# J-Schoepplenberg/zero-packet

Measured on AMD Instinct MI355X. Metric: device-resident Mpkt/s + GB/s, PacketParser::parse, 64-1500B mix, higher is better.
Workload: dtype u8; 1 GPU; 16M IPv4 TCP/UDP/ICMPv4, U[64,1500]B (config 3); config=c3, frames_per_gpu=16777216, bytes_per_gpu=13113571179, job_frames=16777216, job_bytes=13113571179, parallelism=dp1 (independent shards, no collective)

## Files before the change

__graft_entry__.py:

```python
import importlib
import json
import os
import subprocess
import sys

ROOT = os.path.dirname(os.path.abspath(__file__))
PKG = os.path.join(ROOT, "zero-packet_amd")
CSRC = os.path.join(PKG, "csrc")
HIP_SOURCES = ["zp_parse.hip", "zp_parse_slots.hip", "zp_ctx.hip", "zp_gen.hip", "zp_fields.hip", "zp_ring.hip", "zp_build.hip",
               "zp_stats.hip"]
HOST_SOURCES = ["zp_readers.c"]
HIPCC = os.environ.get("HIPCC", "/opt/rocm/bin/hipcc")


def _run(cmd, cwd=ROOT):
    print("+", " ".join(cmd), flush=True)
    subprocess.run(cmd, cwd=cwd, check=True)


def _stale(target, sources):
    if not os.path.exists(target):
        return True
    t = os.path.getmtime(target)
    return any(os.path.getmtime(s) > t for s in sources)


def build(force=False):
    inc = os.path.join(ROOT, "include")
    deps = [os.path.join(CSRC, f) for f in os.listdir(CSRC)] + [
        os.path.join(inc, f) for f in os.listdir(inc)]
    hip_so = os.path.join(PKG, "libzp_hip.so")
    if force or _stale(hip_so, deps):
        objs = []
        for src in HIP_SOURCES:
            obj = os.path.join(CSRC, src.replace(".hip", ".o"))
            _run([HIPCC, "--offload-arch=gfx950", "-O3", "-std=c++17", "-fPIC",
                  "-Wall", "-c", os.path.join(CSRC, src), "-o", obj])
            objs.append(obj)
        for src in HOST_SOURCES:
            obj = os.path.join(CSRC, src.replace(".c", ".o"))
            _run(["gcc", "-O3", "-std=c11", "-Wall", "-Wextra", "-fPIC", "-c",
                  os.path.join(CSRC, src), "-o", obj])
# ... 83 lines not shown
```

include/zero_packet.h:

```cpp
#ifndef ZERO_PACKET_H
#define ZERO_PACKET_H

#include <stddef.h>
#include <stdint.h>

#ifdef __cplusplus
extern "C" {
#endif

#define ZP_ABI_VERSION 6

typedef enum zp_err {
    ZP_OK = 0,
    ZP_ERR_ETH_FRAME_TOO_SHORT = 1,
    ZP_ERR_ETH_SLICE_TOO_SHORT = 2,
    ZP_ERR_ETH_VLAN_TOO_SHORT = 3,
    ZP_ERR_ETH_QINQ_TOO_SHORT = 4,
    ZP_ERR_ETH_INVALID_QINQ = 5,
    ZP_ERR_ARP_TOO_SHORT = 6,
    ZP_ERR_ARP_INVALID_OPER = 7,
    ZP_ERR_IPV4_TOO_SHORT = 8,
    ZP_ERR_IPV4_VERSION = 9,
    ZP_ERR_IPV4_IHL_TOO_SHORT = 10,
    ZP_ERR_IPV4_HDR_TOO_LONG = 11,
// ... 90 lines not shown
        (((c >> 10) & 3u) + 1u) * 8u};
    uint32_t at = 0;
    for (int k = 0; k < ZP_EXT_SLOTS; ++k) x->off[k] = 0;
    for (int j = 0; j < 6; ++j) {
        const int k = order[j];
        if (r.flags & ZP_F_EXT_SLOT(k)) { x->off[k] = (uint16_t)at; at += len[k]; }
    }
    x->len = (uint16_t)at;
    x->final_nh = (uint8_t)((r.flags & ZP_F_TCP) ? 6 : (r.flags & ZP_F_UDP) ? 17
                          : (r.flags & ZP_F_ICMPV4) ? 1 : 58);
    x->reserved = 0;
}

typedef struct zp_rec_fields {
    uint32_t flags;
    uint8_t  err, eth_len, final_nh, inner_final_nh;
    uint32_t inner_off, l4_off;
} zp_rec_fields;

int zp_rec_decode(const zp_record* rec, const uint8_t* frame, uint64_t len,
                  const zp_ext_offsets* ext, zp_rec_fields* out);

int zp_abi_version(void);
const char* zp_err_str(int code);
const char* zp_last_error(void);

int zp_parse_batch_device(const uint8_t* arena, const uint64_t* offs,
                          const uint32_t* lens, uint64_t n,
                          zp_record* records, zp_ext_offsets* ext,
                          void* stream);

int zp_set_record_slots(int mode);
int zp_record_slots_state(void);

typedef struct zp_ctx zp_ctx;
zp_ctx* zp_ctx_create(int device, uint64_t chunk_bytes);
void    zp_ctx_destroy(zp_ctx* ctx);
int zp_parse_batch_host(zp_ctx* ctx, const uint8_t* arena, uint64_t arena_bytes,
                        const uint64_t* offs, const uint32_t* lens, uint64_t n,
                        zp_record* records, zp_ext_offsets* ext);
int zp_parse_batch_host_multi(zp_ctx* const* ctxs, int nctx, const uint8_t* arena,
                              uint64_t arena_bytes, const uint64_t* offs,
                              const uint32_t* lens, uint64_t n, zp_record* records,
                              zp_ext_offsets* ext);
int zp_parse_one(zp_ctx* ctx, const uint8_t* frame, uint64_t len,
                 zp_record* record, zp_ext_offsets ext[2]);
int zp_parse_one_config(zp_ctx* ctx, uint32_t idle_us);
int zp_device_current(void);

typedef enum zp_reader_kind {
    ZP_READER_ETHERNET = 0,
    ZP_READER_ARP = 1,
    ZP_READER_IPV4 = 2,
    ZP_READER_IPV6 = 3,
    ZP_READER_OPTIONS = 4,
    ZP_READER_ROUTING = 5,
    ZP_READER_FRAGMENT = 6,
    ZP_READER_AUTH = 7,
    ZP_READER_TCP = 8,
    ZP_READER_UDP = 9,
    ZP_READER_ICMPV4 = 10,
    ZP_READER_ICMPV6 = 11,
    ZP_READER_KIND_COUNT = 12
} zp_reader_kind;

typedef struct zp_reader_info {
// ... 204 lines not shown
```

zero-packet_amd/_lib.py:

```python
import ctypes
import os

HERE = os.path.dirname(os.path.abspath(__file__))
HIP_LIB = os.path.join(HERE, "libzp_hip.so")
HOST_LIB = os.path.join(HERE, "libzp_host.so")

_hip = None
_pyhip = None
_host = None

c_u8p = ctypes.c_void_p


def _sig(lib, name, res, args):
    f = getattr(lib, name)
    f.restype = res
    f.argtypes = args
    return f


def hip():
    global _hip
    if _hip is None:
        if not os.path.exists(HIP_LIB):
            raise RuntimeError(f"zero-packet_amd: HIP library missing ({HIP_LIB}); "
                               "run __graft_entry__.build() - there is no CPU fallback")
        lib = ctypes.CDLL(HIP_LIB)
        vp, u64, u32, i32 = ctypes.c_void_p, ctypes.c_uint64, ctypes.c_uint32, ctypes.c_int
        _sig(lib, "zp_abi_version", i32, [])
        _sig(lib, "zp_err_str", ctypes.c_char_p, [i32])
        _sig(lib, "zp_last_error", ctypes.c_char_p, [])
        _sig(lib, "zp_parse_batch_device", i32, [vp, vp, vp, u64, vp, vp, vp])
        _sig(lib, "zp_set_record_slots", i32, [i32])
        _sig(lib, "zp_record_slots_state", i32, [])
        _sig(lib, "zp_ctx_create", vp, [i32, u64])
        _sig(lib, "zp_ctx_destroy", None, [vp])
        _sig(lib, "zp_parse_batch_host", i32, [vp, vp, u64, vp, vp, u64, vp, vp])
        _sig(lib, "zp_parse_batch_host_multi", i32, [vp, i32, vp, u64, vp, vp, u64, vp, vp])
        _sig(lib, "zp_parse_one", i32, [vp, vp, u64, vp, vp])
        _sig(lib, "zp_parse_one_config", i32, [vp, u32])
        _sig(lib, "zp_device_current", i32, [])
        _sig(lib, "zp__one_test_hooks", i32, [vp, u32, u64, u32])
        _sig(lib, "zp__one_stats", i32, [vp, vp])
        _sig(lib, "zp_col_width", i32, [i32])
        _sig(lib, "zp_build_err_str", ctypes.c_char_p, [i32])
        _sig(lib, "zp_build_batch_device", i32, [vp, vp, vp, u64, vp, vp, vp, vp, vp])
        _sig(lib, "zp_extract_columns_device", i32, [vp, vp, vp, vp, u64, vp, vp])
        _sig(lib, "zp_parse_batch_columns_device", i32, [vp, vp, vp, u64, vp, vp, vp, vp])
        _sig(lib, "zp_stats_device", i32, [vp, u64, vp, vp])
        _sig(lib, "zp_probe_read_device", i32, [vp, u64, vp, vp])
        _sig(lib, "zp_probe_tiles_device", i32, [vp, u64, u64, vp, vp, vp, vp, vp])
        _sig(lib, "zp_probe_tiles_codes_device", i32, [vp, u64, u64, vp, vp, vp, vp, vp])
        _sig(lib, "zp_gen_lengths_device", i32, [i32, u64, u64, u64, vp, vp])
        _sig(lib, "zp_gen_frames_device", i32, [i32, u64, u64, u64, vp, vp, vp, vp])
        _sig(lib, "zp_reader_new", i32, [i32, vp, u64, vp])
        _sig(lib, "zp_internet_checksum", ctypes.c_uint16, [vp, u64, u32])
        _sig(lib, "zp_verify_internet_checksum", i32, [vp, u64, u32])
        _sig(lib, "zp_pseudo_header", u32, [vp, vp, u32, ctypes.c_uint8, u64])
        _sig(lib, "zp_rec_decode", i32, [vp, vp, u64, vp, vp])
        _hip = lib
    return _hip


def pyhip():
    global _pyhip
    if _pyhip is None:
        hip()
# ... 27 lines not shown
```

zero-packet_amd/csrc/zp_parse.hip:

```cpp

#include <hip/hip_runtime.h>
#include <stdint.h>
#include <string.h>
#include <stdio.h>
#include <stdlib.h>
#include <mutex>

#include "../../include/zero_packet.h"
#include "../../include/zero_packet_errstr.h"
#include "zp_cols.h"
#define ZP_WIN 112
#define ZP_WPE 5
#include "zp_stream.h"

#define ZP_WAVES 1
#define ZP_EXT_DENSE 32
#define ZP_K 1
#define ZP_SMALL_G 4
#define ZP_TAIL_G 4

#ifndef ZP_PARSE_SLOTS_TU
static __thread char g_last_error[256];

static void set_err(const char* what, hipError_t e) {
    snprintf(g_last_error, sizeof g_last_error, "%s: %s", what, hipGetErrorString(e));
}

extern "C" const char* zp_last_error(void) { return g_last_error; }
extern "C" __attribute__((visibility("hidden"))) char* zp__errbuf(void) { return g_last_error; }
extern "C" int zp_abi_version(void) { return ZP_ABI_VERSION; }
extern "C" const char* zp_err_str(int code) { return zp_err_string(code); }
#endif


__device__ __forceinline__ bool icmpv4_type_ok(uint32_t t) {
    const uint64_t m0 = (1ull << 0) | (1ull << 3) | (1ull << 4) | (1ull << 5) | (1ull << 8) |
                        (1ull << 9) | (1ull << 10) | (1ull << 11) | (1ull << 12) | (1ull << 13) |
                        (1ull << 14) | (1ull << 15) | (1ull << 16) | (1ull << 17) | (1ull << 18) |
                        (1ull << 30) | (1ull << 40) | (1ull << 42) | (1ull << 43);
    if (t < 64) return (m0 >> t) & 1;
    return t == 253 || t == 254;
}
__device__ __forceinline__ bool icmpv6_type_ok(uint32_t t) {
    if (t >= 1 && t <= 4) return true;
    if (t == 100 || t == 101 || t == 155 || t == 200 || t == 201) return true;
    return t >= 128 && t <= 153;
}

#define ZP_RSTRIDE (ZP_WIN / 4 + 1)
struct FrameView {
    const uint4* win;
    const uint32_t* reg;
    bool region;
    const uint8_t* g;
// ... 558 lines not shown

template <bool COLS, bool SYS = false, class L = WaveLds, bool SLOTS = false>
__device__ __forceinline__ void tile_finish(TileState& s, uint64_t n, int lane, L& lds,
                                            zp_record* __restrict__ records,
                                            zp_ext_offsets* __restrict__ ext,
                                            const ColPtrs& cols, uintptr_t sysbase = 0,
                                            zp_u32x2* sys_rec = nullptr) {
    constexpr bool TAILS = sizeof(lds.win) > sizeof(uint4) * ZP_WIN_CH * 64;
    static_assert(TAILS || !SYS, "the tail-free layout needs the region path");
    uint4* tail = TAILS ? &lds.win[0] + ZP_WIN_CH * 64 : nullptr;
    const uint8_t* g = (const uint8_t*)s.ga;
    const uint32_t fsum = lds.cend[s.rank & 63u] - ((s.rank & 63u) ? lds.cend[(s.rank & 63u) - 1u] : 0u);
    FrameView fv;
    fv.win = &lds.win[0];
    fv.g = g;
    fv.lane = s.rank & 63u;
    fv.shift = s.shift;
    fv.len = s.len;
    fv.wlen = s.wlen;
    fv.xc = make_uint4(0, 0, 0, 0);
    fv.xi = ~0u;
    fv.sysbase = SYS ? sysbase : 0;
    uint4 mytail;
    fv.region = !SYS;
    if (SYS) {
        mytail = tail[s.rank & 63u];
        fv.reg = nullptr;
    } else {
        static_assert(64 * ZP_RSTRIDE * 4 <= sizeof(L), "regions fit the wave's LDS");
        const uint32_t rk = s.rank & 63u;
        uint4 cell[ZP_WIN_CH];
#pragma unroll
        for (uint32_t c = 0; c < ZP_WIN_CH; ++c) cell[c] = lds.win[c * 64 + ((rk ^ c) & 63u)];
        mytail = tail[rk];
        wave_lds_fence();
        uint32_t* reg = (uint32_t*)&lds.win[0] + (uint32_t)lane * ZP_RSTRIDE;
#pragma unroll
        for (uint32_t c = 0; c < ZP_WIN_CH; ++c) {
            reg[4 * c] = cell[c].x; reg[4 * c + 1] = cell[c].y;
            reg[4 * c + 2] = cell[c].z; reg[4 * c + 3] = cell[c].w;
        }
        wave_lds_fence();
        fv.reg = reg;
    }
    Walk w;
    w.rec = zp_rec_full{};
    w.outer = make_uint4(0, 0, 0, 0);
    w.inner = make_uint4(0, 0, 0, 0);
    bool done = false;
    const Probe pr = probe_frame(fv);
    const bool probe = s.live && v4_probe(fv, pr);
    if (__builtin_popcountll(__ballot(probe)) >= (SYS ? 1 : 32)) {
        if (probe) done = fast_v4(fv, pr, w);
    }
    {
        const bool todo = s.live && !done;
        if (__ballot(todo) && !__ballot(todo && !fast_ip_probe(fv, pr))) {
            if (todo) done = fast_ip(fv, pr, w);
        }
    }
    if (__ballot(s.live && !done)) {
        if (s.live && !done) {
            w.rec = zp_rec_full{};
            walk_frame(fv, w);
        }
    }
    if (!s.live) return;
// ... 33 lines not shown
        const bool ho = (rec.flags & ZP_F_EXT) && !zp_chain_inline(rec),
                   hi = rec.flags & ZP_F_INNER_EXT;
        const uint64_t mo = __ballot(ho), mi = __ballot(hi);
        if (SYS) {
            if (ho) st_sys16(sysbase, (uintptr_t)(ext + p),
                             zp_u32x4{w.outer.x, w.outer.y, w.outer.z, w.outer.w});
            if (hi) st_sys16(sysbase, (uintptr_t)(ext + n + p),
                             zp_u32x4{w.inner.x, w.inner.y, w.inner.z, w.inner.w});
            if (ho || hi) asm volatile("s_waitcnt vmcnt(0)" ::: "memory");
        } else {
        if (mo && (ho || __builtin_popcountll(mo) >= ZP_EXT_DENSE))
            store_ext(ext, p, ho ? w.outer : make_uint4(0, 0, 0, 0));
        if (mi && (hi || __builtin_popcountll(mi) >= ZP_EXT_DENSE))
            store_ext(ext, n + p, hi ? w.inner : make_uint4(0, 0, 0, 0));
        }
    }
    if (COLS) {
        ViewReader rdr{fv};
        emit_columns(rdr, rec, rec.err == 0 && (rec.flags & ZP_F_ETHERNET), s.len, p, cols);
    }
}


#define ZP_KATTR __launch_bounds__(64 * ZP_WAVES) __attribute__((amdgpu_waves_per_eu(ZP_WPE)))
#define ZP_KATTR_COLS __launch_bounds__(64 * ZP_WAVES)
template <bool COLS, bool TINY = !COLS, class L = WaveLds, bool SLOTS = false>
__device__ __forceinline__ void parse_tile(uint64_t t, uint32_t len, uintptr_t ga, uint64_t n,
                                           int lane, L& lds,
                                           zp_record* __restrict__ records,
                                           zp_ext_offsets* __restrict__ ext,
                                           const ColPtrs& cols) {
    const uintptr_t fallback = (uintptr_t)&zp_safe_chunk;
    uint4* win = &lds.win[0];
    uint4* tail = &lds.win[0] + ZP_WIN_CH * 64;
    if (TINY && !__ballot(t * 64 + lane < n && len != 64u) &&
        tiny_tile(t, len, ga, n, lane, records, SLOTS))
        return;
    TileState s;
    tile_setup(s, t, len, ga, n, lane, lds);
    if (s.nitems <= ZP_SMALL_G) {
        uint4 vs[ZP_SMALL_G];
        uint32_t ks[ZP_SMALL_G];
        issue_group<ZP_SMALL_G>(0, s.nitems, s.cur, s.R, lane, fallback, vs, ks);
        consume_group<ZP_SMALL_G>(0, s.nitems, lane, vs, ks, win, tail, lds.cend, s.run);
    } else
    {
    uint4 va[ZP_G];
    uint32_t ka[ZP_G];
    issue_group<ZP_G>(0, s.nitems, s.cur, s.R, lane, fallback, va, ka);
    consume_group<ZP_G>(0, s.nitems, lane, va, ka, win, tail, lds.cend, s.run);
    for (uint32_t i0 = ZP_G; i0 < s.nitems; i0 += ZP_G) {
        if (s.nitems - i0 <= 2) {
            uint4 vt[2];
            uint32_t kt[2];
            issue_group<2>(i0, s.nitems, s.cur, s.R, lane, fallback, vt, kt);
            consume_group<2>(i0, s.nitems, lane, vt, kt, win, tail, lds.cend, s.run);
            break;
        }
        if (s.nitems - i0 <= ZP_TAIL_G) {
            uint4 vt[ZP_TAIL_G];
            uint32_t kt[ZP_TAIL_G];
            issue_group<ZP_TAIL_G>(i0, s.nitems, s.cur, s.R, lane, fallback, vt, kt);
            consume_group<ZP_TAIL_G>(i0, s.nitems, lane, vt, kt, win, tail, lds.cend, s.run);
            break;
        }
        issue_group<ZP_G>(i0, s.nitems, s.cur, s.R, lane, fallback, va, ka);
        consume_group<ZP_G>(i0, s.nitems, lane, va, ka, win, tail, lds.cend, s.run);
    }
    }
    wave_lds_fence();
    {
        const uint32_t r = s.rank & 63u;
        const uintptr_t org = ((uintptr_t)bperm(s.R.org_hi, r) << 32) | bperm(s.R.org_lo, r);
        s.ga = org + 16ull * bperm(s.R.pfx, r) + s.shift;
    }
    __builtin_amdgcn_s_setprio(0);
    tile_finish<COLS, false, L, SLOTS>(s, n, lane, lds, records, ext, cols);
}

template <bool COLS, bool SLOTS = false>
__device__ __forceinline__ void parse_tiles(const uint8_t* __restrict__ arena,
                                            const uint64_t* __restrict__ offs,
                                            const uint32_t* __restrict__ lens, uint64_t n,
                                            zp_record* __restrict__ records,
                                            zp_ext_offsets* __restrict__ ext,
                                            const ColPtrs& cols) {
    __shared__ WaveLds lds_all[ZP_WAVES];
    const int lane = threadIdx.x & 63;
    const int wid = threadIdx.x >> 6;
    WaveLds& lds = lds_all[wid];
    const uint64_t blk = blockIdx.x;
    for (uint32_t k = 0; k < ZP_K; ++k) {
        const uint64_t t = (blk * ZP_WAVES + wid) * ZP_K + k;
        if (t * 64 >= n) return;
        __builtin_amdgcn_s_setprio(1);
        if (k) wave_lds_fence();
        uint32_t len;
        uintptr_t ga;
        load_desc(arena, offs, lens, n, t, lane, len, ga);
        parse_tile<COLS, !COLS, WaveLds, SLOTS>(t, len, ga, n, lane, lds, records, ext, cols);
    }
}

#ifdef ZP_PARSE_SLOTS_TU
__global__ void ZP_KATTR
zp_parse_slots_kernel(const uint8_t* __restrict__ arena, const uint64_t* __restrict__ offs,
                      const uint32_t* __restrict__ lens, uint64_t n,
                      zp_record* __restrict__ records, zp_ext_offsets* __restrict__ ext) {
    const ColPtrs none{};
    parse_tiles<false, true>(arena, offs, lens, n, records, ext, none);
}
extern "C" __attribute__((visibility("hidden"))) hipError_t
zp__parse_slots_launch(uint64_t blocks, hipStream_t stream, const uint8_t* arena, const uint64_t* offs,
                       const uint32_t* lens, uint64_t n, zp_record* records, zp_ext_offsets* ext) {
    hipLaunchKernelGGL(zp_parse_slots_kernel, dim3((unsigned)blocks), dim3(64 * ZP_WAVES), 0, stream,
                       arena, offs, lens, n, records, ext);
    return hipGetLastError();
}
#else
extern "C" hipError_t zp__parse_slots_launch(uint64_t blocks, hipStream_t stream, const uint8_t* arena,
                                             const uint64_t* offs, const uint32_t* lens, uint64_t n,
                                             zp_record* records, zp_ext_offsets* ext);
__global__ void ZP_KATTR
zp_parse_kernel(const uint8_t* __restrict__ arena, const uint64_t* __restrict__ offs,
                const uint32_t* __restrict__ lens, uint64_t n,
                zp_record* __restrict__ records, zp_ext_offsets* __restrict__ ext) {
    const ColPtrs none{};
    parse_tiles<false>(arena, offs, lens, n, records, ext, none);
}

#define ZP_EXPAND_TILES 16
__global__ void __launch_bounds__(256) zp_rec_expand_kernel(zp_record* __restrict__ records, uint64_t n,
                                                             uint32_t* __restrict__ hint, uint32_t token) {
    const uint32_t lane = threadIdx.x & 63u;
    const uint64_t t0 = ((uint64_t)blockIdx.x * 4 + (threadIdx.x >> 6)) * ZP_EXPAND_TILES;
    const uint64_t full = n / 64;
    const uint32_t b3 = lane < ZP_EXPAND_TILES && t0 + lane < full
// ... 2 lines not shown
    if (!m) return;
    if (hint && lane == 0 && (threadIdx.x >> 6) == 0 && (blockIdx.x & 63u) == 0 &&
        __builtin_popcountll(m) * 4 >= 3 * ZP_EXPAND_TILES)
        __hip_atomic_store(hint, token, __ATOMIC_RELAXED, __HIP_MEMORY_SCOPE_SYSTEM);
    uint32_t c[ZP_EXPAND_TILES];
#pragma unroll
    for (int k = 0; k < ZP_EXPAND_TILES; ++k)
        c[k] = (m >> k) & 1u ? ((const uint8_t*)(records + (t0 + k) * 64))[lane] : 0u;
#pragma unroll
    for (int k = 0; k < ZP_EXPAND_TILES; ++k)
        if ((m >> k) & 1u)
            __builtin_nontemporal_store(code_rec(c[k]), (zp_u32x2*)(records + (t0 + k) * 64 + lane));
}

extern "C" __attribute__((visibility("hidden"))) int zp__rec_expand_launch(zp_record* records, uint64_t n,
                                                                         hipStream_t stream,
                                                                         uint32_t* hint, uint32_t token) {
    if (n < 64) return 0;
    const uint64_t per_block = 4 * ZP_EXPAND_TILES;
    hipLaunchKernelGGL(zp_rec_expand_kernel, dim3((unsigned)((n / 64 + per_block - 1) / per_block)),
                       dim3(256), 0, stream, records, n, hint, token);
    const hipError_t e = hipGetLastError();
    if (e != hipSuccess) { set_err("zp_rec_expand_kernel launch", e); return -2; }
    return 0;
}

#define ZP_SLOT_MIN_FRAMES (1ull << 21)
static int g_slot_mode = 0;
extern "C" int zp_set_record_slots(int mode) {
    if (mode < 0 || mode > 2) return -1;
    return __atomic_exchange_n(&g_slot_mode, mode, __ATOMIC_RELAXED);
}

#define ZP_SLOT_PROBE_EVERY 16
struct SlotState {
    std::mutex mu;
    uint32_t* word = nullptr;
    uint32_t* word_d = nullptr;
    hipEvent_t ev = nullptr;
    bool pending = false, decision = true, broken = false;
    uint64_t since = 0;
    uint64_t last_n = 0;
    uint32_t token = 0;
};
static SlotState g_slot_state[64];

extern "C" int zp_record_slots_state(void) {
    int dev = 0;
    if (hipGetDevice(&dev) != hipSuccess) { (void)hipGetLastError(); dev = 0; }
    SlotState& st = g_slot_state[dev & 63];
    std::lock_guard<std::mutex> guard(st.mu);
    return st.decision ? 1 : 0;
}

static bool slot_state_init(SlotState& st) {
    if (st.word || st.broken) return !st.broken;
    void* w = nullptr;
    if (hipHostMalloc(&w, 64, hipHostMallocMapped | hipHostMallocCoherent) != hipSuccess ||
        hipHostGetDevicePointer((void**)&st.word_d, w, 0) != hipSuccess ||
        hipEventCreateWithFlags(&st.ev, hipEventDisableTiming) != hipSuccess) {
        (void)hipGetLastError();
        st.broken = true;
        return false;
    }
    st.word = (uint32_t*)w;
    return true;
}

__global__ void ZP_KATTR_COLS
zp_parse_columns_kernel(const uint8_t* __restrict__ arena, const uint64_t* __restrict__ offs,
                        const uint32_t* __restrict__ lens, uint64_t n,
                        zp_record* __restrict__ records, zp_ext_offsets* __restrict__ ext,
                        ColPtrs cols) {
    parse_tiles<true>(arena, offs, lens, n, records, ext, cols);
}

extern "C" int zp_parse_batch_device(const uint8_t* arena, const uint64_t* offs,
                                     const uint32_t* lens, uint64_t n,
                                     zp_record* records, zp_ext_offsets* ext,
                                     void* stream) {
    if (n == 0) return 0;
    if (!arena || !offs || !lens || !records) {
        snprintf(g_last_error, sizeof g_last_error, "zp_parse_batch_device: null pointer");
        return -1;
    }
    const uint64_t per_block = 64ull * ZP_WAVES * ZP_K;
    const uint64_t blocks = (n + per_block - 1) / per_block;
    if (blocks > 0x7FFFFFFFull) {
        snprintf(g_last_error, sizeof g_last_error, "zp_parse_batch_device: batch too large");
        return -1;
    }
    const int mode = __atomic_load_n(&g_slot_mode, __ATOMIC_RELAXED);
    const hipStream_t st_h = (hipStream_t)stream;
    auto launch = [&](bool slots, uint32_t* hint, uint32_t token) -> int {
        hipError_t e;
        if (slots) {
            e = zp__parse_slots_launch(blocks, st_h, arena, offs, lens, n, records, ext);
        } else {
            hipLaunchKernelGGL(zp_parse_kernel, dim3((unsigned)blocks), dim3(64 * ZP_WAVES), 0,
                               st_h, arena, offs, lens, n, records, ext);
            e = hipGetLastError();
        }
        if (e != hipSuccess) { set_err("zp_parse_kernel launch", e); return -2; }
        return slots ? zp__rec_expand_launch(records, n, st_h, hint, token) : 0;
    };
    if (mode != 0 || n < ZP_SLOT_MIN_FRAMES) return launch(mode == 1, nullptr, 0);
    int dev = 0;
    if (hipGetDevice(&dev) != hipSuccess) { (void)hipGetLastError(); dev = 0; }
    SlotState& st = g_slot_state[dev & 63];
    std::lock_guard<std::mutex> guard(st.mu);
    hipStreamCaptureStatus cs = hipStreamCaptureStatusNone;
    if (hipStreamIsCapturing(st_h, &cs) != hipSuccess) { (void)hipGetLastError(); cs = hipStreamCaptureStatusActive; }
    if (cs != hipStreamCaptureStatusNone) return launch(st.decision, nullptr, 0);
    if (n != st.last_n) {
        st.last_n = n;
        st.since = 0;
        st.pending = false;
    }
    if (st.pending) {
        const hipError_t q = hipEventQuery(st.ev);
        if (q == hipSuccess) {
            st.decision = __atomic_load_n(st.word, __ATOMIC_ACQUIRE) == st.token;
            st.pending = false;
        } else {
            (void)hipGetLastError();
        }
    }
    if (st.pending || st.since++ % ZP_SLOT_PROBE_EVERY != 0 || !slot_state_init(st))
        return launch(st.decision, nullptr, 0);
    st.token = st.token + 1 ? st.token + 1 : 1;
    const int rc = launch(true, st.word_d, st.token);
    if (rc == 0 && hipEventRecord(st.ev, st_h) == hipSuccess) st.pending = true;
    else (void)hipGetLastError();
    return rc;
}

extern "C" int zp_parse_batch_columns_device(const uint8_t* arena, const uint64_t* offs,
                                             const uint32_t* lens, uint64_t n,
                                             zp_record* records, zp_ext_offsets* ext,
                                             void* const* cols, void* stream) {
    if (n == 0) return 0;
    if (!arena || !offs || !lens || !records || !cols) {
        snprintf(g_last_error, sizeof g_last_error, "zp_parse_batch_columns_device: null pointer");
        return -1;
    }
    ColPtrs c;
    for (int k = 0; k < ZP_COL_COUNT; ++k) c.p[k] = (uint8_t*)cols[k];
    const uint64_t per_block = 64ull * ZP_WAVES * ZP_K;
    const uint64_t blocks = (n + per_block - 1) / per_block;
    if (blocks > 0x7FFFFFFFull) {
        snprintf(g_last_error, sizeof g_last_error, "zp_parse_batch_columns_device: batch too large");
        return -1;
    }
    hipLaunchKernelGGL(zp_parse_columns_kernel, dim3((unsigned)blocks), dim3(64 * ZP_WAVES), 0,
                       (hipStream_t)stream, arena, offs, lens, n, records, ext, c);
    const hipError_t e = hipGetLastError();
    if (e != hipSuccess) { set_err("zp_parse_columns_kernel launch", e); return -2; }
    return 0;
}

#define ZP_ONE_BELL 0
#define ZP_ONE_REC 64
#define ZP_ONE_ACK 72
#define ZP_ONE_EXT 96
// ... 124 lines not shown
```

zero-packet_amd/csrc/zp_stream.h:

```cpp
#pragma once
#include <hip/hip_runtime.h>
#include <stdint.h>

#ifndef ZP_WIN
#define ZP_WIN 128
#endif
#define ZP_WIN_CH (ZP_WIN / 16)
static_assert(ZP_WIN % 16 == 0 && ZP_WIN <= 256, "ZP_WIN must be a multiple of 16, <= 256");
#define ZP_GIANT 65536u
#define ZP_G 8

#define ZP_GLOBAL __attribute__((address_space(1)))
typedef unsigned zp_u32x4 __attribute__((ext_vector_type(4)));
typedef unsigned zp_u32x2 __attribute__((ext_vector_type(2)));

__device__ __forceinline__ uint4 ldg16(uintptr_t a) {
    zp_u32x4 v = *(const ZP_GLOBAL zp_u32x4*)a;
    return make_uint4(v.x, v.y, v.z, v.w);
}
__device__ __forceinline__ uint32_t ldg4(uintptr_t a) { return *(const ZP_GLOBAL uint32_t*)a; }

__device__ __forceinline__ uint4 ld_stream(uintptr_t a) {
    zp_u32x4 v = __builtin_nontemporal_load((const ZP_GLOBAL zp_u32x4*)a);
    return make_uint4(v.x, v.y, v.z, v.w);
// ... 84 lines not shown
        s = sad16(d[i] & m, s);
    }
    return s;
}

struct Cursor {
    uint32_t rbase;
    uint32_t nz;
    uint64_t* starts;
};

struct Ranked {
    uint32_t org_lo, org_hi;
    uint32_t last;
    uint32_t pfx;
    uint32_t mid;
};

#define KEEP_IN (1u << 31)
#define KEEP_WIN (1u << 30)
#define KEEP_TAIL (1u << 29)
#define ZP_T4N 3
#define KEEP_T4 (1u << 28)
#define KEEP_T4D(k) (((k) >> 22) & 3u)
#define KEEP_MID (1u << 27)
#define KEEP_MIDB(k) (((k) >> 10) & 15u)
#define KEEP_CELL(k) ((k) & 0x3FFu)
#define KEEP_RANK(k) (((k) >> 16) & 63u)

__device__ __forceinline__ uint32_t bperm(uint32_t v, uint32_t r) {
    return (uint32_t)__builtin_amdgcn_ds_bpermute((int)(r << 2), (int)v);
}

#define ZP_STARTS 64
__device__ __forceinline__ void build_starts(uint32_t w0, const Cursor& c, const Ranked& R,
                                             int lane) {
    if ((uint32_t)lane < (uint32_t)ZP_STARTS) c.starts[lane] = 0;
    __builtin_amdgcn_fence(__ATOMIC_RELEASE, "wavefront");
    __builtin_amdgcn_wave_barrier();
    __builtin_amdgcn_fence(__ATOMIC_ACQUIRE, "wavefront");
    const uint32_t it = R.pfx >> 6;
    if ((uint32_t)lane < c.nz && it >= w0 && it < w0 + (uint32_t)ZP_STARTS)
        __hip_atomic_fetch_or(&c.starts[it - w0], 1ull << (R.pfx & 63u), __ATOMIC_RELAXED,
                              __HIP_MEMORY_SCOPE_WAVEFRONT);
    __builtin_amdgcn_fence(__ATOMIC_RELEASE, "wavefront");
    __builtin_amdgcn_wave_barrier();
    __builtin_amdgcn_fence(__ATOMIC_ACQUIRE, "wavefront");
}

template <int G, bool T4 = false>
__device__ __forceinline__ void issue_group(uint32_t i0, uint32_t nitems, Cursor& c,
                                            const Ranked& R, int lane, uintptr_t fallback,
                                            uint4 (&v)[G], uint32_t (&keep)[G]) {
    uintptr_t a[G];
    static_assert(ZP_STARTS % G == 0 && G % 2 == 0 && ZP_STARTS <= 64,
                  "group size must be even and divide ZP_STARTS");
    if ((i0 & (ZP_STARTS - 1u)) == 0 && i0 < nitems) build_starts(i0, c, R, lane);
    uint64_t Fq[G];
    zp_u32x4 m[G / 2];
    const zp_u32x4* sp = (const zp_u32x4*)&c.starts[i0 & (ZP_STARTS - 1u)];
#pragma unroll
    for (int q = 0; q < G / 2; ++q) m[q] = sp[q];
#pragma unroll
    for (int q = 0; q < G; ++q) {
        const uint32_t lo = (q & 1) ? m[q / 2].z : m[q / 2].x;
        const uint32_t hi = (q & 1) ? m[q / 2].w : m[q / 2].y;
        const uint64_t fu = ((uint64_t)(uint32_t)__builtin_amdgcn_readfirstlane(hi) << 32) |
// ... 35 lines not shown
__device__ __forceinline__ void retire_group(const uint4 (&v)[G]) {
#pragma unroll
    for (int q = 0; q < G; ++q) asm volatile("" ::"v"(v[q].x), "v"(v[q].y), "v"(v[q].z), "v"(v[q].w));
}

template <int G, bool T4 = false>
__device__ __forceinline__ void consume_group(uint32_t i0, uint32_t nitems, int lane,
                                              const uint4 (&v)[G], const uint32_t (&keep)[G],
                                              uint4* win, uint4* tail, uint32_t* cend,
                                              uint32_t& run, uint4* t4 = nullptr,
                                              uint32_t* cmid = nullptr) {
#pragma unroll
    for (int q = 0; q < G; ++q) {
        const uint32_t i = i0 + q;
        if (i >= nitems) continue;
        const uint32_t k = keep[q];
        if (k & KEEP_WIN) win[KEEP_CELL(k)] = v[q];
        if (T4 && (k & KEEP_T4)) t4[KEEP_RANK(k) * ZP_T4N + KEEP_T4D(k)] = v[q];
        uint32_t part = sad16(v[q].x, 0u);
        part = sad16(v[q].y, part);
        part = sad16(v[q].z, part);
        part = sad16(v[q].w, part);
        const uint32_t P = wave_scan(k & KEEP_IN ? part : 0u);
        if (k & KEEP_TAIL) {
            if (tail != nullptr) tail[KEEP_RANK(k)] = v[q];
            cend[KEEP_RANK(k)] = run + P;
        }
        if (T4 && (k & KEEP_MID)) cmid[KEEP_RANK(k)] = run + P - part + range_sum(v[q], 0u, KEEP_MIDB(k));
        run += rdl(P, 63);
    }
    retire_group(v);
}

struct WaveLds {
    uint4 win[(ZP_WIN_CH + 1) * 64];
    uint32_t cend[64];
    uint64_t starts[ZP_STARTS];
};

struct TileState {
    uint64_t tile;
    uintptr_t ga;
    uint32_t len, shift, wlen, rank;
    bool live, giant;
    uint32_t nitems;
    uint64_t ranked;
    Ranked R;
    Cursor cur;
    uint32_t run;
};

template <class L>
__device__ __forceinline__ void tile_setup(TileState& s, uint64_t tile, uint32_t len,
                                           uintptr_t ga, uint64_t n, int lane, L& lds,
                                           bool win_only = false, uint32_t mark = ~0u) {
    s.tile = tile;
    s.ga = ga;
    s.len = len;
    s.live = tile * 64 + lane < n;
    s.shift = (uint32_t)(ga & 15);
    s.wlen = len < ZP_WIN - s.shift ? len : ZP_WIN - s.shift;
    s.giant = len > ZP_GIANT;
    const uint32_t span = s.giant || (win_only && len + s.shift > ZP_WIN) ? (uint32_t)ZP_WIN
                                                                          : len + s.shift;
    const uint32_t nch = len >= 64 ? (span + 15) >> 4 : 0u;
    const uint64_t M = __ballot(nch > 0);
    s.ranked = M;
    s.rank = __builtin_amdgcn_mbcnt_hi((uint32_t)(M >> 32),
                                       __builtin_amdgcn_mbcnt_lo((uint32_t)M, 0u));
    const uint32_t incl = wave_scan(nch);
    const uint32_t pfx = incl - nch;
    const uint32_t T = rdl(incl, 63);
    s.nitems = (T + 63) >> 6;
    const uint32_t nz = (uint32_t)__builtin_popcountll(M);
    const uint32_t dst = nch ? s.rank : nz + ((uint32_t)lane - s.rank);
    const uintptr_t org = (ga & ~(uintptr_t)15) - 16ull * pfx;
    const int a = (int)(dst << 2);
    s.R.org_lo = (uint32_t)__builtin_amdgcn_ds_permute(a, (int)(uint32_t)org);
    s.R.org_hi = (uint32_t)__builtin_amdgcn_ds_permute(a, (int)(uint32_t)(org >> 32));
    s.R.last = (uint32_t)__builtin_amdgcn_ds_permute(a, (int)(incl - 1));
    s.R.pfx = (uint32_t)__builtin_amdgcn_ds_permute(a, (int)pfx);
    const uint32_t mc = mark != ~0u && nch ? (s.shift + mark) >> 4 : ~0u;
    const uint32_t mid = mc < nch ? ((pfx + mc) << 4) | ((s.shift + mark) & 15u) : ~0u;
    s.R.mid = (uint32_t)__builtin_amdgcn_ds_permute(a, (int)mid);
    s.cur.rbase = ~0u;
    s.cur.nz = nz;
    s.cur.starts = &lds.starts[0];
    s.run = 0;
}

__device__ __forceinline__ void wave_lds_fence() {
    __builtin_amdgcn_fence(__ATOMIC_RELEASE, "wavefront");
    __builtin_amdgcn_wave_barrier();
    __builtin_amdgcn_fence(__ATOMIC_ACQUIRE, "wavefront");
}

__device__ __forceinline__ void load_desc(const uint8_t* arena, const uint64_t* offs,
                                          const uint32_t* lens, uint64_t n, uint64_t tile,
                                          int lane, uint32_t& len, uintptr_t& ga) {
    const uint64_t p = tile * 64 + lane;
    const uint64_t pc = p < n ? p : n - 1;
    const uint32_t l = lens[pc];
    const uint64_t o = offs[pc];
    len = p < n ? l : 0u;
    ga = (uintptr_t)arena + (p < n ? o : 0);
}
```

Before: 8470 Mpkt/s.

## Add tail-free LDS parse variants selected by a sampled batch profile

Adds two kernel variants that drop the per-wave LDS tail buffer, with window sizes 112 or 128 and a smaller starts array. Each frame's last 16-byte chunk is then taken from the neighbouring window cell or reloaded from global memory. A sampling profile kernel checks whether frames are packed contiguously and how often IPv6 extension headers appear, and the host uses that to pick a layout on later calls. The smaller LDS footprint is meant to raise occupancy, at the cost of extra global loads for tails, an extra profiling launch, and more dispatch complexity.

```diff
diff --git a/__graft_entry__.py b/__graft_entry__.py
--- a/__graft_entry__.py
+++ b/__graft_entry__.py
@@ -7,7 +7,7 @@
 ROOT = os.path.dirname(os.path.abspath(__file__))
 PKG = os.path.join(ROOT, "zero-packet_amd")
 CSRC = os.path.join(PKG, "csrc")
-HIP_SOURCES = ["zp_parse.hip", "zp_parse_slots.hip", "zp_ctx.hip", "zp_gen.hip", "zp_fields.hip", "zp_ring.hip", "zp_build.hip",
+HIP_SOURCES = ["zp_parse.hip", "zp_parse_slots.hip", "zp_parse_tf.hip", "zp_parse_tf128.hip", "zp_ctx.hip", "zp_gen.hip", "zp_fields.hip", "zp_ring.hip", "zp_build.hip",
                "zp_stats.hip"]
 HOST_SOURCES = ["zp_readers.c"]
 HIPCC = os.environ.get("HIPCC", "/opt/rocm/bin/hipcc")
diff --git a/include/zero_packet.h b/include/zero_packet.h
--- a/include/zero_packet.h
+++ b/include/zero_packet.h
@@ -146,6 +146,8 @@
 
 int zp_set_record_slots(int mode);
 int zp_record_slots_state(void);
+int zp_set_parse_layout(int mode);
+int zp_parse_layout_state(void);
 
 typedef struct zp_ctx zp_ctx;
 zp_ctx* zp_ctx_create(int device, uint64_t chunk_bytes);
diff --git a/zero-packet_amd/_lib.py b/zero-packet_amd/_lib.py
--- a/zero-packet_amd/_lib.py
+++ b/zero-packet_amd/_lib.py
@@ -33,6 +33,8 @@
         _sig(lib, "zp_parse_batch_device", i32, [vp, vp, vp, u64, vp, vp, vp])
         _sig(lib, "zp_set_record_slots", i32, [i32])
         _sig(lib, "zp_record_slots_state", i32, [])
+        _sig(lib, "zp_set_parse_layout", i32, [i32])
+        _sig(lib, "zp_parse_layout_state", i32, [])
         _sig(lib, "zp_ctx_create", vp, [i32, u64])
         _sig(lib, "zp_ctx_destroy", None, [vp])
         _sig(lib, "zp_parse_batch_host", i32, [vp, vp, u64, vp, vp, u64, vp, vp])
diff --git a/zero-packet_amd/csrc/zp_parse.hip b/zero-packet_amd/csrc/zp_parse.hip
--- a/zero-packet_amd/csrc/zp_parse.hip
+++ b/zero-packet_amd/csrc/zp_parse.hip
@@ -9,9 +9,17 @@
 #include "../../include/zero_packet.h"
 #include "../../include/zero_packet_errstr.h"
 #include "zp_cols.h"
+#ifndef ZP_WIN
 #define ZP_WIN 112
+#endif
 #define ZP_WPE 5
+#ifndef ZP_DESC_NT
+#define ZP_DESC_NT 0
+#endif
 #include "zp_stream.h"
+#if defined(ZP_PARSE_SLOTS_TU) || defined(ZP_PARSE_TF_TU)
+#define ZP_PARSE_KERNEL_TU 1
+#endif
 
 #define ZP_WAVES 1
 #define ZP_EXT_DENSE 32
@@ -19,7 +27,7 @@
 #define ZP_SMALL_G 4
 #define ZP_TAIL_G 4
 
-#ifndef ZP_PARSE_SLOTS_TU
+#ifndef ZP_PARSE_KERNEL_TU
 static __thread char g_last_error[256];
 
 static void set_err(const char* what, hipError_t e) {
@@ -644,7 +652,18 @@
         uint4 cell[ZP_WIN_CH];
 #pragma unroll
         for (uint32_t c = 0; c < ZP_WIN_CH; ++c) cell[c] = lds.win[c * 64 + ((rk ^ c) & 63u)];
-        mytail = tail[rk];
+        if (TAILS) {
+            mytail = tail[rk];
+        } else {
+            const uint32_t nr = (rk + 1u) & 63u;
+            const uint4 ncell = lds.win[nr];
+            const uintptr_t nA = ((((uintptr_t)bperm(s.R.org_hi, nr)) << 32) | bperm(s.R.org_lo, nr)) +
+                                 16ull * bperm(s.R.pfx, nr);
+            const uintptr_t lastc = (s.ga + s.len - 1u) & ~(uintptr_t)15;
+            const bool nxt = rk + 1u < s.cur.nz && nA == lastc;
+            const bool need = s.live && s.len >= 64 && !s.giant && ((s.len + s.shift) & 15u) != 0u;
+            mytail = nxt ? ncell : (need ? ldg16(lastc) : make_uint4(0, 0, 0, 0));
+        }
         wave_lds_fence();
         uint32_t* reg = (uint32_t*)&lds.win[0] + (uint32_t)lane * ZP_RSTRIDE;
 #pragma unroll
@@ -744,7 +763,8 @@
                                            const ColPtrs& cols) {
     const uintptr_t fallback = (uintptr_t)&zp_safe_chunk;
     uint4* win = &lds.win[0];
-    uint4* tail = &lds.win[0] + ZP_WIN_CH * 64;
+    uint4* tail = sizeof(lds.win) > sizeof(uint4) * ZP_WIN_CH * 64 ? &lds.win[0] + ZP_WIN_CH * 64
+                                                                  : nullptr;
     if (TINY && !__ballot(t * 64 + lane < n && len != 64u) &&
         tiny_tile(t, len, ga, n, lane, records, SLOTS))
         return;
@@ -790,17 +810,17 @@
     tile_finish<COLS, false, L, SLOTS>(s, n, lane, lds, records, ext, cols);
 }
 
-template <bool COLS, bool SLOTS = false>
+template <bool COLS, bool SLOTS = false, class L = WaveLds>
 __device__ __forceinline__ void parse_tiles(const uint8_t* __restrict__ arena,
                                             const uint64_t* __restrict__ offs,
                                             const uint32_t* __restrict__ lens, uint64_t n,
                                             zp_record* __restrict__ records,
                                             zp_ext_offsets* __restrict__ ext,
                                             const ColPtrs& cols) {
-    __shared__ WaveLds lds_all[ZP_WAVES];
+    __shared__ L lds_all[ZP_WAVES];
     const int lane = threadIdx.x & 63;
     const int wid = threadIdx.x >> 6;
-    WaveLds& lds = lds_all[wid];
+    L& lds = lds_all[wid];
     const uint64_t blk = blockIdx.x;
     for (uint32_t k = 0; k < ZP_K; ++k) {
         const uint64_t t = (blk * ZP_WAVES + wid) * ZP_K + k;
@@ -809,12 +829,27 @@
         if (k) wave_lds_fence();
         uint32_t len;
         uintptr_t ga;
-        load_desc(arena, offs, lens, n, t, lane, len, ga);
-        parse_tile<COLS, !COLS, WaveLds, SLOTS>(t, len, ga, n, lane, lds, records, ext, cols);
-    }
-}
-
-#ifdef ZP_PARSE_SLOTS_TU
+        load_desc<ZP_DESC_NT != 0>(arena, offs, lens, n, t, lane, len, ga);
+        parse_tile<COLS, !COLS, L, SLOTS>(t, len, ga, n, lane, lds, records, ext, cols);
+    }
+}
+
+#if defined(ZP_PARSE_TF_TU)
+__global__ void ZP_KATTR
+ZP_TF_KERNEL(const uint8_t* __restrict__ arena, const uint64_t* __restrict__ offs,
+             const uint32_t* __restrict__ lens, uint64_t n,
+             zp_record* __restrict__ records, zp_ext_offsets* __restrict__ ext) {
+    const ColPtrs none{};
+    parse_tiles<false, false, WaveLdsTailFree>(arena, offs, lens, n, records, ext, none);
+}
+extern "C" __attribute__((visibility("hidden"))) hipError_t
+ZP_TF_LAUNCH(uint64_t blocks, hipStream_t stream, const uint8_t* arena, const uint64_t* offs,
+             const uint32_t* lens, uint64_t n, zp_record* records, zp_ext_offsets* ext) {
+    hipLaunchKernelGGL(ZP_TF_KERNEL, dim3((unsigned)blocks), dim3(64 * ZP_WAVES), 0, stream,
+                       arena, offs, lens, n, records, ext);
+    return hipGetLastError();
+}
+#elif defined(ZP_PARSE_SLOTS_TU)
 __global__ void ZP_KATTR
 zp_parse_slots_kernel(const uint8_t* __restrict__ arena, const uint64_t* __restrict__ offs,
                       const uint32_t* __restrict__ lens, uint64_t n,
@@ -883,37 +918,143 @@
     return __atomic_exchange_n(&g_slot_mode, mode, __ATOMIC_RELAXED);
 }
 
+static int g_layout_mode = 0;
+extern "C" int zp_set_parse_layout(int mode) {
+    if (mode == -1) return __atomic_load_n(&g_layout_mode, __ATOMIC_RELAXED);
+    if (mode < 0 || mode > 3) return -1;
+    return __atomic_exchange_n(&g_layout_mode, mode, __ATOMIC_RELAXED);
+}
+extern "C" hipError_t zp__parse_tf_launch(uint64_t blocks, hipStream_t stream, const uint8_t* arena,
+                                          const uint64_t* offs, const uint32_t* lens, uint64_t n,
+                                          zp_record* records, zp_ext_offsets* ext);
+extern "C" hipError_t zp__parse_tf128_launch(uint64_t blocks, hipStream_t stream, const uint8_t* arena,
+                                             const uint64_t* offs, const uint32_t* lens, uint64_t n,
+                                             zp_record* records, zp_ext_offsets* ext);
+
+#define ZP_PROFILE_STRIDE 64
+#define ZP_PROFILE_PER_WAVE 4
+#define ZP_PROFILE_WAVES 16
+#define ZP_PROFILE_ACC_WORDS 8
+#define ZP_PROFILE_OUT 4
+__global__ void __launch_bounds__(64 * ZP_PROFILE_WAVES)
+zp_batch_profile_kernel(const uint8_t* __restrict__ arena, const uint64_t* __restrict__ offs,
+                        const uint32_t* __restrict__ lens, uint64_t n, uint32_t* __restrict__ acc,
+                        uint32_t* __restrict__ out, uint32_t token) {
+    __shared__ unsigned long long sums[ZP_PROFILE_WAVES][2];
+    const uint32_t lane = threadIdx.x & 63u, wave = threadIdx.x >> 6;
+    unsigned long long A = 0, B = 0;
+#pragma unroll
+    for (int j = 0; j < ZP_PROFILE_PER_WAVE; ++j) {
+        const uint64_t smp = ((uint64_t)blockIdx.x * ZP_PROFILE_WAVES + wave) * ZP_PROFILE_PER_WAVE + j;
+        const uint64_t p0 = smp * ZP_PROFILE_STRIDE * 64;
+        if (p0 >= n) break;
+        const uint64_t p = p0 + lane;
+        const bool live = p < n;
+        const uint64_t pc = live ? p : n - 1;
+        const uint64_t o = offs[pc];
+        const uint32_t len = lens[pc];
+        const bool pair = lane < 63 && p + 1 < n;
+        const uint64_t o1 = offs[pair ? p + 1 : pc];
+        const bool packed = !__ballot(pair && o + len != o1);
+        const uint8_t* f = arena + o;
+        auto at = [&](uint32_t i) -> uint32_t { return live && i < len && i < 32u ? f[i] : 0x100u; };
+        const uint32_t t0 = at(12) << 8 | at(13);
+        const uint32_t hl = t0 == 0x8100 ? 18u : t0 == 0x88A8 ? 22u : 14u;
+        const uint32_t et = hl == 14u ? t0 : at(hl - 2) << 8 | at(hl - 1);
+        const uint32_t nh = at(hl + 6);
+        const bool v6ext = et == 0x86DD && (nh == 0 || nh == 43 || nh == 44 || nh == 51 || nh == 60);
+        A += (1ull << 32) | (packed ? 1ull : 0ull);
+        B += ((unsigned long long)__builtin_popcountll(__ballot(live)) << 32) |
+             (unsigned long long)__builtin_popcountll(__ballot(v6ext));
+    }
+    if (lane == 0) { sums[wave][0] = A; sums[wave][1] = B; }
+    __syncthreads();
+    if (threadIdx.x != 0) return;
+    A = B = 0;
+    for (int w = 0; w < ZP_PROFILE_WAVES; ++w) { A += sums[w][0]; B += sums[w][1]; }
+    unsigned long long* a64 = (unsigned long long*)(acc + (token & 3u) * ZP_PROFILE_ACC_WORDS);
+    uint32_t* done = (uint32_t*)(a64 + 2);
+    atomicAdd(a64, A);
+    atomicAdd(a64 + 1, B);
+    __threadfence();
+    if (atomicAdd(done, 1u) + 1u != gridDim.x) return;
+    __threadfence();
+    A = atomicExch(a64, 0ull);
+    B = atomicExch(a64 + 1, 0ull);
+    atomicExch(done, 0u);
+    uint64_t* o64 = (uint64_t*)(out + ZP_PROFILE_OUT);
+    __hip_atomic_store(o64, (uint64_t)A, __ATOMIC_RELAXED, __HIP_MEMORY_SCOPE_SYSTEM);
+    __hip_atomic_store(o64 + 1, (uint64_t)B, __ATOMIC_RELAXED, __HIP_MEMORY_SCOPE_SYSTEM);
+    __hip_atomic_store(out + ZP_PROFILE_OUT + 4, token, __ATOMIC_RELEASE, __HIP_MEMORY_SCOPE_SYSTEM);
+}
+
 #define ZP_SLOT_PROBE_EVERY 16
-struct SlotState {
+#define ZP_PROFILE_V6EXT_DEN 2
+struct BatchProfile {
     std::mutex mu;
     uint32_t* word = nullptr;
     uint32_t* word_d = nullptr;
+    uint32_t* acc_d = nullptr;
     hipEvent_t ev = nullptr;
     bool pending = false, decision = true, broken = false;
+    bool probed_codes = false, probed_layout = false;
+    int layout = 1;
     uint64_t since = 0;
     uint64_t last_n = 0;
     uint32_t token = 0;
 };
-static SlotState g_slot_state[64];
-
-extern "C" int zp_record_slots_state(void) {
+static BatchProfile g_profile[64];
+
+static void profile_poll(BatchProfile& st) {
+    if (!st.pending) return;
+    if (hipEventQuery(st.ev) != hipSuccess) {
+        (void)hipGetLastError();
+        return;
+    }
+    st.pending = false;
+    if (st.probed_codes) st.decision = __atomic_load_n(st.word, __ATOMIC_ACQUIRE) == st.token;
+    if (st.probed_layout &&
+        __atomic_load_n(st.word + ZP_PROFILE_OUT + 4, __ATOMIC_ACQUIRE) == st.token) {
+        uint64_t s[2];
+        memcpy(s, st.word + ZP_PROFILE_OUT, sizeof s);
+        const uint64_t tiles = s[0] >> 32, packed = s[0] & 0xFFFFFFFFull;
+        const uint64_t frames = s[1] >> 32, exts = s[1] & 0xFFFFFFFFull;
+        st.layout = packed != tiles ? 1 : exts * ZP_PROFILE_V6EXT_DEN >= frames ? 3 : 2;
+    }
+}
+
+static BatchProfile& profile_here(void) {
     int dev = 0;
     if (hipGetDevice(&dev) != hipSuccess) { (void)hipGetLastError(); dev = 0; }
-    SlotState& st = g_slot_state[dev & 63];
+    return g_profile[dev & 63];
+}
+
+extern "C" int zp_record_slots_state(void) {
+    BatchProfile& st = profile_here();
     std::lock_guard<std::mutex> guard(st.mu);
+    profile_poll(st);
     return st.decision ? 1 : 0;
 }
-
-static bool slot_state_init(SlotState& st) {
+extern "C" int zp_parse_layout_state(void) {
+    BatchProfile& st = profile_here();
+    std::lock_guard<std::mutex> guard(st.mu);
+    profile_poll(st);
+    return st.layout;
+}
+
+static bool profile_init(BatchProfile& st) {
     if (st.word || st.broken) return !st.broken;
     void* w = nullptr;
     if (hipHostMalloc(&w, 64, hipHostMallocMapped | hipHostMallocCoherent) != hipSuccess ||
         hipHostGetDevicePointer((void**)&st.word_d, w, 0) != hipSuccess ||
+        hipMalloc((void**)&st.acc_d, 4 * ZP_PROFILE_ACC_WORDS * sizeof(uint32_t)) != hipSuccess ||
+        hipMemset(st.acc_d, 0, 4 * ZP_PROFILE_ACC_WORDS * sizeof(uint32_t)) != hipSuccess ||
         hipEventCreateWithFlags(&st.ev, hipEventDisableTiming) != hipSuccess) {
         (void)hipGetLastError();
         st.broken = true;
         return false;
     }
+    memset(w, 0, 64);
     st.word = (uint32_t*)w;
     return true;
 }
@@ -942,11 +1083,16 @@
         return -1;
     }
     const int mode = __atomic_load_n(&g_slot_mode, __ATOMIC_RELAXED);
+    const int lmode = __atomic_load_n(&g_layout_mode, __ATOMIC_RELAXED);
     const hipStream_t st_h = (hipStream_t)stream;
-    auto launch = [&](bool slots, uint32_t* hint, uint32_t token) -> int {
+    auto launch = [&](bool slots, int layout, uint32_t* hint, uint32_t token) -> int {
         hipError_t e;
         if (slots) {
             e = zp__parse_slots_launch(blocks, st_h, arena, offs, lens, n, records, ext);
+        } else if (layout == 2) {
+            e = zp__parse_tf_launch(blocks, st_h, arena, offs, lens, n, records, ext);
+        } else if (layout == 3) {
+            e = zp__parse_tf128_launch(blocks, st_h, arena, offs, lens, n, records, ext);
         } else {
             hipLaunchKernelGGL(zp_parse_kernel, dim3((unsigned)blocks), dim3(64 * ZP_WAVES), 0,
                                st_h, arena, offs, lens, n, records, ext);
@@ -955,32 +1101,37 @@
         if (e != hipSuccess) { set_err("zp_parse_kernel launch", e); return -2; }
         return slots ? zp__rec_expand_launch(records, n, st_h, hint, token) : 0;
     };
-    if (mode != 0 || n < ZP_SLOT_MIN_FRAMES) return launch(mode == 1, nullptr, 0);
-    int dev = 0;
-    if (hipGetDevice(&dev) != hipSuccess) { (void)hipGetLastError(); dev = 0; }
-    SlotState& st = g_slot_state[dev & 63];
+    if ((mode != 0 && lmode != 0) || n < ZP_SLOT_MIN_FRAMES)
+        return launch(mode == 1, lmode ? lmode : 1, nullptr, 0);
+    BatchProfile& st = profile_here();
     std::lock_guard<std::mutex> guard(st.mu);
+    auto decided = [&](void) -> int {
+        return launch(mode ? mode == 1 : st.decision, lmode ? lmode : st.layout, nullptr, 0);
+    };
     hipStreamCaptureStatus cs = hipStreamCaptureStatusNone;
     if (hipStreamIsCapturing(st_h, &cs) != hipSuccess) { (void)hipGetLastError(); cs = hipStreamCaptureStatusActive; }
-    if (cs != hipStreamCaptureStatusNone) return launch(st.decision, nullptr, 0);
+    if (cs != hipStreamCaptureStatusNone) return decided();
     if (n != st.last_n) {
         st.last_n = n;
         st.since = 0;
         st.pending = false;
     }
-    if (st.pending) {
-        const hipError_t q = hipEventQuery(st.ev);
-        if (q == hipSuccess) {
-            st.decision = __atomic_load_n(st.word, __ATOMIC_ACQUIRE) == st.token;
-            st.pending = false;
-        } else {
-            (void)hipGetLastError();
-        }
-    }
-    if (st.pending || st.since++ % ZP_SLOT_PROBE_EVERY != 0 || !slot_state_init(st))
-        return launch(st.decision, nullptr, 0);
+    profile_poll(st);
+    if (st.pending || st.since++ % ZP_SLOT_PROBE_EVERY != 0 || !profile_init(st)) return decided();
     st.token = st.token + 1 ? st.token + 1 : 1;
-    const int rc = launch(true, st.word_d, st.token);
+    st.probed_codes = mode == 0;
+    st.probed_layout = lmode == 0 && mode != 1 && (mode == 2 || !st.decision || st.since == 1);
+    int rc = launch(mode ? mode == 1 : true, lmode ? lmode : st.layout,
+                    mode == 0 ? st.word_d : nullptr, st.token);
+    if (rc == 0 && st.probed_layout) {
+        const uint64_t samples = ((n + 63) / 64 + ZP_PROFILE_STRIDE - 1) / ZP_PROFILE_STRIDE;
+        const uint64_t per_wg = ZP_PROFILE_WAVES * ZP_PROFILE_PER_WAVE;
+        hipLaunchKernelGGL(zp_batch_profile_kernel, dim3((unsigned)((samples + per_wg - 1) / per_wg)),
+                           dim3(64 * ZP_PROFILE_WAVES), 0, st_h, arena, offs, lens, n, st.acc_d,
+                           st.word_d, st.token);
+        const hipError_t e = hipGetLastError();
+        if (e != hipSuccess) { set_err("zp_batch_profile_kernel launch", e); rc = -2; }
+    }
     if (rc == 0 && hipEventRecord(st.ev, st_h) == hipSuccess) st.pending = true;
     else (void)hipGetLastError();
     return rc;
diff --git a/zero-packet_amd/csrc/zp_parse_tf.hip b/zero-packet_amd/csrc/zp_parse_tf.hip
--- /dev/null
+++ b/zero-packet_amd/csrc/zp_parse_tf.hip
@@ -0,0 +1,6 @@
+#define ZP_PARSE_TF_TU 1
+#define ZP_TF_KERNEL zp_parse_tf_kernel
+#define ZP_TF_LAUNCH zp__parse_tf_launch
+#define ZP_WIN 112
+#define ZP_STARTS 32
+#include "zp_parse.hip"
diff --git a/zero-packet_amd/csrc/zp_parse_tf128.hip b/zero-packet_amd/csrc/zp_parse_tf128.hip
--- /dev/null
+++ b/zero-packet_amd/csrc/zp_parse_tf128.hip
@@ -0,0 +1,6 @@
+#define ZP_PARSE_TF_TU 1
+#define ZP_TF_KERNEL zp_parse_tf128_kernel
+#define ZP_TF_LAUNCH zp__parse_tf128_launch
+#define ZP_WIN 128
+#define ZP_STARTS 32
+#include "zp_parse.hip"
diff --git a/zero-packet_amd/csrc/zp_stream.h b/zero-packet_amd/csrc/zp_stream.h
--- a/zero-packet_amd/csrc/zp_stream.h
+++ b/zero-packet_amd/csrc/zp_stream.h
@@ -140,7 +140,9 @@
     return (uint32_t)__builtin_amdgcn_ds_bpermute((int)(r << 2), (int)v);
 }
 
+#ifndef ZP_STARTS
 #define ZP_STARTS 64
+#endif
 __device__ __forceinline__ void build_starts(uint32_t w0, const Cursor& c, const Ranked& R,
                                              int lane) {
     if ((uint32_t)lane < (uint32_t)ZP_STARTS) c.starts[lane] = 0;
@@ -242,11 +244,14 @@
     retire_group(v);
 }
 
-struct WaveLds {
-    uint4 win[(ZP_WIN_CH + 1) * 64];
+template <int TAILS>
+struct WaveLdsT {
+    uint4 win[(ZP_WIN_CH + TAILS) * 64];
     uint32_t cend[64];
     uint64_t starts[ZP_STARTS];
 };
+typedef WaveLdsT<1> WaveLds;
+typedef WaveLdsT<0> WaveLdsTailFree;
 
 struct TileState {
     uint64_t tile;
@@ -305,13 +310,14 @@
     __builtin_amdgcn_fence(__ATOMIC_ACQUIRE, "wavefront");
 }
 
+template <bool NT = false>
 __device__ __forceinline__ void load_desc(const uint8_t* arena, const uint64_t* offs,
                                           const uint32_t* lens, uint64_t n, uint64_t tile,
                                           int lane, uint32_t& len, uintptr_t& ga) {
     const uint64_t p = tile * 64 + lane;
     const uint64_t pc = p < n ? p : n - 1;
-    const uint32_t l = lens[pc];
-    const uint64_t o = offs[pc];
+    const uint32_t l = NT ? __builtin_nontemporal_load(lens + pc) : lens[pc];
+    const uint64_t o = NT ? __builtin_nontemporal_load(offs + pc) : offs[pc];
     len = p < n ? l : 0u;
     ga = (uintptr_t)arena + (p < n ? o : 0);
 }
```

Measured after the change: 8424 Mpkt/s. No clear change (-0.5%).
